# ZhicengShi/mclSTExp

Hardware: AMD Instinct MI355X
Metric: training spots/sec (= steps/sec x global batch) at batch 128/GPU, 224px patches, 1000 genes (higher is better)
Workload: dtype bf16; 1 GPU; BASELINE configs[1]: train step, batch 128/GPU, 224x224 patches, 1000 genes, densenet121 image encoder; global_batch=128, parallelism=dp1, backbone_dtype=bf16, infonce=fused, infonce_effective=exact (fused from 1024 pairs), hip_graphs=True, optimizer=Adam(lr=1e-4, wd=1e-3) incl. 2x(65536,G) tables

## Files before the change

mclstexp_amd/csrc/dense_bwd.hip:

```cpp
#include "common.h"
#include <stdlib.h>

namespace {

constexpr int TN = 128, TK = 128;

template <int MODE, int TMv>
__global__ __launch_bounds__(256, (TMv == 64 && MODE != 2 ? 3 : 2)) void bn1_bwd_kernel(const bf16_t* __restrict__ dz, const bf16_t* __restrict__ W1,
                                                         int K , int ldw ,
                                                         const bf16_t* __restrict__ x, long long ldx, long long S,
                                                         const float* __restrict__ gamma,
                                                         const float* __restrict__ beta,
                                                         const float* __restrict__ mean,
                                                         const float* __restrict__ rstd,
                                                         const float* __restrict__ coef ,
                                                         bf16_t* gbuf, long long ldg,
                                                         float2* __restrict__ partial , int nrt) {
  __shared__ __attribute__((aligned(16))) unsigned char lds[TK * 256 + TMv * 256 + 2048];
  const int tid = threadIdx.x, lane = tid & 63, wave = tid >> 6;
  const int h = lane >> 5, l31 = lane & 31;
  const int wm = wave >> 1, wn = wave & 1;
  const int n0 = blockIdx.y * TN;
  unsigned char* wt = lds;
  unsigned char* dzt = lds + TK * 256;
  bf16_t* xt = reinterpret_cast<bf16_t*>(dzt);
  float* red = reinterpret_cast<float*>(lds + TK * 256 + TMv * 256);

  const int cc = tid & 15, rr = tid >> 4;
  const bool cok = n0 + cc * 8 < K;
  constexpr int NL = TMv / 16, RI = TMv / 64;
  uint4 dzr[NL], xr[NL], gr[NL];
  auto issue_loads = [&](int rt) {
    const long long row0 = (long long)rt * TMv;
#pragma unroll
    for (int i = 0; i < NL; ++i) {
      const long long rg = row0 + rr + 16 * i;
      const bool ok = rg < S;
      dzr[i] = ok ? *reinterpret_cast<const uint4*>(dz + rg * TK + cc * 8) : make_uint4(0u, 0u, 0u, 0u);
      xr[i] = (ok && cok) ? *reinterpret_cast<const uint4*>(x + rg * ldx + n0 + cc * 8) : make_uint4(0u, 0u, 0u, 0u);
      if (MODE >= 1)
        gr[i] = (ok && cok) ? *reinterpret_cast<const uint4*>(gbuf + rg * ldg + n0 + cc * 8) : make_uint4(0u, 0u, 0u, 0u);
    }
  };
  if ((int)blockIdx.x < nrt) issue_loads(blockIdx.x);
  {
    uint4 wv[8];
#pragma unroll
    for (int i = 0; i < 8; ++i) {
      const int k = rr + 16 * i;
      wv[i] = cok ? *reinterpret_cast<const uint4*>(W1 + (long long)k * ldw + n0 + cc * 8) : make_uint4(0u, 0u, 0u, 0u);
    }
#pragma unroll
    for (int i = 0; i < 8; ++i) {
      const int k = rr + 16 * i;
      const int f = ((k & 3) << 2) | ((k >> 2) & 3);
      *reinterpret_cast<uint4*>(wt + k * 256 + ((cc ^ f) << 4)) = wv[i];
    }
  }
  float mu[2], rs[2], sc[2], sh[2], c1[2], c2[2];
#pragma unroll
  for (int j = 0; j < 2; ++j) {
    const int c = n0 + wn * 64 + j * 32 + l31;
    const bool cvalid = c < K;
    mu[j] = cvalid ? mean[c] : 0.0f;
    rs[j] = cvalid ? rstd[c] : 0.0f;
    sc[j] = cvalid ? gamma[c] * rs[j] : 0.0f;
    sh[j] = cvalid ? fmaf(-mu[j], sc[j], beta[c]) : 0.0f;
    c1[j] = (MODE >= 1 && coef != nullptr && cvalid) ? coef[2 * c] : 0.0f;
    c2[j] = (MODE >= 1 && coef != nullptr && cvalid) ? coef[2 * c + 1] : 0.0f;
  }
  const int q = (lane & 15) >> 2, jj = lane & 3;
  const int g2 = 2 * ((lane >> 4) & 1) + (jj >> 1);

  for (int rt = blockIdx.x; rt < nrt; rt += gridDim.x) {
    const long long row0 = (long long)rt * TMv;
    if (rt != (int)blockIdx.x) issue_loads(rt);
    __syncthreads();
#pragma unroll
    for (int i = 0; i < NL; ++i) {
      const int r = rr + 16 * i;
      *reinterpret_cast<uint4*>(dzt + r * 256 + ((cc ^ (r & 15)) << 4)) = dzr[i];
    }
    __syncthreads();

    f32x16 acc[RI][2];
#pragma unroll
    for (int i = 0; i < RI; ++i)
#pragma unroll
      for (int j = 0; j < 2; ++j)
#pragma unroll
        for (int r = 0; r < 16; ++r) acc[i][j][r] = 0.0f;
#pragma unroll
    for (int ks = 0; ks < 8; ++ks) {
      bf16x8 fa[RI], fb[2];
#pragma unroll
      for (int i = 0; i < RI; ++i) {
        const int r = wm * (TMv / 2) + i * 32 + l31;
        fa[i] = *reinterpret_cast<const bf16x8*>(dzt + r * 256 + (((2 * ks + h) ^ (r & 15)) << 4));
      }
#pragma unroll
      for (int j = 0; j < 2; ++j) {
        const int chunk = (wn * 64 + j * 32) / 8 + g2;
        const int k_lo = 16 * ks + 8 * h + q, k_hi = k_lo + 4;
        const int f_lo = ((k_lo & 3) << 2) | ((k_lo >> 2) & 3), f_hi = ((k_hi & 3) << 2) | ((k_hi >> 2) & 3);
        const v4s lo = __builtin_amdgcn_ds_read_tr16_b64_v4i16(
            (v4s __attribute__((address_space(3)))*)(wt + k_lo * 256 + ((chunk ^ f_lo) << 4) + (jj & 1) * 8));
        const v4s hi = __builtin_amdgcn_ds_read_tr16_b64_v4i16(
            (v4s __attribute__((address_space(3)))*)(wt + k_hi * 256 + ((chunk ^ f_hi) << 4) + (jj & 1) * 8));
        fb[j][0] = lo[0]; fb[j][1] = lo[1]; fb[j][2] = lo[2]; fb[j][3] = lo[3];
        fb[j][4] = hi[0]; fb[j][5] = hi[1]; fb[j][6] = hi[2]; fb[j][7] = hi[3];
      }
#pragma unroll
      for (int i = 0; i < RI; ++i)
#pragma unroll
        for (int j = 0; j < 2; ++j) acc[i][j] = __builtin_amdgcn_mfma_f32_32x32x16_bf16(fa[i], fb[j], acc[i][j], 0, 0, 0);
    }
    __syncthreads();
#pragma unroll
    for (int i = 0; i < NL; ++i) *reinterpret_cast<uint4*>(xt + (rr + 16 * i) * TN + cc * 8) = xr[i];
    __syncthreads();

    const long long nvalid = min((long long)TMv, S - row0);
    float s1[2], s2[2];
#pragma unroll
    for (int j = 0; j < 2; ++j) {
      const int cl = wn * 64 + j * 32 + l31;
      s1[j] = s2[j] = 0.0f;
      const float ka = MODE == 2 ? -c2[j] * rs[j] : -sc[j] * c2[j] * rs[j];
      const float kb = fmaf(-ka, mu[j], MODE == 2 ? -c1[j] : -sc[j] * c1[j]);
#pragma unroll
      for (int i = 0; i < RI; ++i)
#pragma unroll
        for (int r = 0; r < 16; ++r) {
          const int row = wm * (TMv / 2) + i * 32 + (r & 3) + 8 * (r >> 2) + 4 * h;
          const float xv = bf2f(xt[row * TN + cl]);
          const float gi = fmaf(xv, sc[j], sh[j]) > 0.0f ? acc[i][j][r] : 0.0f;
          if (MODE != 1) {
            if (row < nvalid) {
              s1[j] += gi;
              s2[j] = fmaf(gi, xv, s2[j]);
            }
          }
          if (MODE >= 1) xt[row * TN + cl] = f2bf(fmaf(sc[j], gi, fmaf(ka, xv, kb)));
        }
      if (MODE != 1) s2[j] = rs[j] * fmaf(-mu[j], s1[j], s2[j]);
    }
    if (MODE != 1) {
#pragma unroll
      for (int j = 0; j < 2; ++j) {
        s1[j] += __shfl_xor(s1[j], 32, 64);
        s2[j] += __shfl_xor(s2[j], 32, 64);
        if (h == 0) {
          const int cl = wn * 64 + j * 32 + l31;
          red[(wm * 128 + cl) * 2] = s1[j];
          red[(wm * 128 + cl) * 2 + 1] = s2[j];
        }
      }
      __syncthreads();
      if (tid < 128 && n0 + tid < K)
        partial[(long long)(n0 + tid) * nrt + rt] = make_float2(red[tid * 2] + red[(128 + tid) * 2],
                                                                red[tid * 2 + 1] + red[(128 + tid) * 2 + 1]);
    }
    if (MODE >= 1) {
      if (MODE == 1) __syncthreads();
      if (cok) {
#pragma unroll
        for (int i = 0; i < NL; ++i) {
          const int r = rr + 16 * i;
          const long long rg = row0 + r;
          if (rg < S) {
            const uint4 dv = *reinterpret_cast<const uint4*>(xt + r * TN + cc * 8);
            const unsigned gw[4] = {gr[i].x, gr[i].y, gr[i].z, gr[i].w}, dw[4] = {dv.x, dv.y, dv.z, dv.w};
            unsigned o[4];
#pragma unroll
            for (int u = 0; u < 4; ++u) {
              const float lo = __uint_as_float(gw[u] << 16) + __uint_as_float(dw[u] << 16);
              const float hi = __uint_as_float(gw[u] & 0xFFFF0000u) + __uint_as_float(dw[u] & 0xFFFF0000u);
              const f32x2 pv = {lo, hi};
              o[u] = __builtin_bit_cast(unsigned, __builtin_convertvector(pv, bf16x2_t));
            }
            *reinterpret_cast<uint4*>(gbuf + rg * ldg + n0 + cc * 8) = make_uint4(o[0], o[1], o[2], o[3]);
          }
        }
      }
    }
  }
}

constexpr size_t PAIR_LDS = 2 * TK * 256 + 64 * 256;
__global__ __launch_bounds__(256, 2) void bn1_dx_pair_kernel(const bf16_t* __restrict__ dzA, const bf16_t* __restrict__ W1A, int ldwA,
                                                             const float* __restrict__ gammaA, const float* __restrict__ betaA,
                                                             const float* __restrict__ coefA, const bf16_t* __restrict__ dzB,
                                                             const bf16_t* __restrict__ W1B, const float* __restrict__ gammaB,
                                                             const float* __restrict__ betaB, const float* __restrict__ coefB,
                                                             int K, const bf16_t* __restrict__ x, long long ldx, long long S,
                                                             const float* __restrict__ mean, const float* __restrict__ rstd,
                                                             bf16_t* gbuf, long long ldg, int nrt) {
  constexpr int TMv = 64;
  extern __shared__ __attribute__((aligned(16))) unsigned char lds[];
  const int tid = threadIdx.x, lane = tid & 63, wave = tid >> 6;
  const int h = lane >> 5, l31 = lane & 31;
  const int wm = wave >> 1, wn = wave & 1;
  const int n0 = blockIdx.y * TN;
  unsigned char* wtA = lds;
  unsigned char* wtB = lds + TK * 256;
  unsigned char* dzt = lds + 2 * TK * 256;
  bf16_t* xt = reinterpret_cast<bf16_t*>(dzt);
  const int cc = tid & 15, rr = tid >> 4;
  const bool cok = n0 + cc * 8 < K;
  constexpr int NL = TMv / 16;
  uint4 dar[NL], dbr[NL], xr[NL], gr[NL];
  auto issue_loads = [&](int rt) {
    const long long row0 = (long long)rt * TMv;
#pragma unroll
    for (int i = 0; i < NL; ++i) {
      const long long rg = row0 + rr + 16 * i;
      const bool ok = rg < S;
      dar[i] = ok ? *reinterpret_cast<const uint4*>(dzA + rg * TK + cc * 8) : make_uint4(0u, 0u, 0u, 0u);
      dbr[i] = ok ? *reinterpret_cast<const uint4*>(dzB + rg * TK + cc * 8) : make_uint4(0u, 0u, 0u, 0u);
      xr[i] = (ok && cok) ? *reinterpret_cast<const uint4*>(x + rg * ldx + n0 + cc * 8) : make_uint4(0u, 0u, 0u, 0u);
      gr[i] = (ok && cok) ? *reinterpret_cast<const uint4*>(gbuf + rg * ldg + n0 + cc * 8) : make_uint4(0u, 0u, 0u, 0u);
    }
  };
  if ((int)blockIdx.x < nrt) issue_loads(blockIdx.x);
  {
    uint4 wa[8], wb[8];
#pragma unroll
    for (int i = 0; i < 8; ++i) {
      const int k = rr + 16 * i;
      wa[i] = cok ? *reinterpret_cast<const uint4*>(W1A + (long long)k * ldwA + n0 + cc * 8) : make_uint4(0u, 0u, 0u, 0u);
      wb[i] = cok ? *reinterpret_cast<const uint4*>(W1B + (long long)k * K + n0 + cc * 8) : make_uint4(0u, 0u, 0u, 0u);
    }
#pragma unroll
    for (int i = 0; i < 8; ++i) {
      const int k = rr + 16 * i;
      const int f = ((k & 3) << 2) | ((k >> 2) & 3);
      *reinterpret_cast<uint4*>(wtA + k * 256 + ((cc ^ f) << 4)) = wa[i];
      *reinterpret_cast<uint4*>(wtB + k * 256 + ((cc ^ f) << 4)) = wb[i];
    }
  }
  float scA[2], shA[2], scB[2], shB[2], ka[2], kb[2];
#pragma unroll
  for (int j = 0; j < 2; ++j) {
    const int c = n0 + wn * 64 + j * 32 + l31;
    const bool cv = c < K;
    const float mu = cv ? mean[c] : 0.0f, rs = cv ? rstd[c] : 0.0f;
    scA[j] = cv ? gammaA[c] * rs : 0.0f;
    shA[j] = cv ? fmaf(-mu, scA[j], betaA[c]) : 0.0f;
    scB[j] = cv ? gammaB[c] * rs : 0.0f;
    shB[j] = cv ? fmaf(-mu, scB[j], betaB[c]) : 0.0f;
    const float c1A = cv ? coefA[2 * c] : 0.0f, c2A = cv ? coefA[2 * c + 1] : 0.0f;
    const float c1B = cv ? coefB[2 * c] : 0.0f, c2B = cv ? coefB[2 * c + 1] : 0.0f;
    const float kaA = -scA[j] * c2A * rs, kaB = -scB[j] * c2B * rs;
    const float kbA = fmaf(-kaA, mu, -scA[j] * c1A), kbB = fmaf(-kaB, mu, -scB[j] * c1B);
    ka[j] = kaA + kaB;
    kb[j] = kbA + kbB;
  }
  const int q = (lane & 15) >> 2, jj = lane & 3;
  const int g2 = 2 * ((lane >> 4) & 1) + (jj >> 1);
  auto product = [&](const unsigned char* wt, f32x16 (&acc)[2]) {
#pragma unroll
    for (int j = 0; j < 2; ++j)
#pragma unroll
      for (int r = 0; r < 16; ++r) acc[j][r] = 0.0f;
#pragma unroll
    for (int ks = 0; ks < 8; ++ks) {
      const int r = wm * (TMv / 2) + l31;
      const bf16x8 fa = *reinterpret_cast<const bf16x8*>(dzt + r * 256 + (((2 * ks + h) ^ (r & 15)) << 4));
      bf16x8 fb[2];
#pragma unroll
      for (int j = 0; j < 2; ++j) {
        const int chunk = (wn * 64 + j * 32) / 8 + g2;
        const int k_lo = 16 * ks + 8 * h + q, k_hi = k_lo + 4;
        const int f_lo = ((k_lo & 3) << 2) | ((k_lo >> 2) & 3), f_hi = ((k_hi & 3) << 2) | ((k_hi >> 2) & 3);
        const v4s lo = __builtin_amdgcn_ds_read_tr16_b64_v4i16(
            (v4s __attribute__((address_space(3)))*)(wt + k_lo * 256 + ((chunk ^ f_lo) << 4) + (jj & 1) * 8));
        const v4s hi = __builtin_amdgcn_ds_read_tr16_b64_v4i16(
            (v4s __attribute__((address_space(3)))*)(wt + k_hi * 256 + ((chunk ^ f_hi) << 4) + (jj & 1) * 8));
        fb[j][0] = lo[0]; fb[j][1] = lo[1]; fb[j][2] = lo[2]; fb[j][3] = lo[3];
        fb[j][4] = hi[0]; fb[j][5] = hi[1]; fb[j][6] = hi[2]; fb[j][7] = hi[3];
      }
#pragma unroll
      for (int j = 0; j < 2; ++j) acc[j] = __builtin_amdgcn_mfma_f32_32x32x16_bf16(fa, fb[j], acc[j], 0, 0, 0);
    }
  };
  for (int rt = blockIdx.x; rt < nrt; rt += gridDim.x) {
    const long long row0 = (long long)rt * TMv;
    if (rt != (int)blockIdx.x) issue_loads(rt);
    __syncthreads();
#pragma unroll
    for (int i = 0; i < NL; ++i) {
      const int r = rr + 16 * i;
      *reinterpret_cast<uint4*>(dzt + r * 256 + ((cc ^ (r & 15)) << 4)) = dar[i];
    }
    __syncthreads();
    f32x16 accA[2], accB[2];
    product(wtA, accA);
    __syncthreads();
#pragma unroll
    for (int i = 0; i < NL; ++i) {
      const int r = rr + 16 * i;
      *reinterpret_cast<uint4*>(dzt + r * 256 + ((cc ^ (r & 15)) << 4)) = dbr[i];
    }
    __syncthreads();
    product(wtB, accB);
    __syncthreads();
#pragma unroll
    for (int i = 0; i < NL; ++i) *reinterpret_cast<uint4*>(xt + (rr + 16 * i) * TN + cc * 8) = xr[i];
    __syncthreads();
#pragma unroll
    for (int j = 0; j < 2; ++j) {
      const int cl = wn * 64 + j * 32 + l31;
#pragma unroll
      for (int r = 0; r < 16; ++r) {
        const int row = wm * (TMv / 2) + (r & 3) + 8 * (r >> 2) + 4 * h;
        const float xv = bf2f(xt[row * TN + cl]);
        const float gA = fmaf(xv, scA[j], shA[j]) > 0.0f ? accA[j][r] : 0.0f;
        const float gB = fmaf(xv, scB[j], shB[j]) > 0.0f ? accB[j][r] : 0.0f;
        xt[row * TN + cl] = f2bf(fmaf(scA[j], gA, fmaf(scB[j], gB, fmaf(ka[j], xv, kb[j]))));
      }
    }
    __syncthreads();
    if (cok) {
#pragma unroll
      for (int i = 0; i < NL; ++i) {
        const int r = rr + 16 * i;
        const long long rg = row0 + r;
        if (rg < S) {
          const uint4 dv = *reinterpret_cast<const uint4*>(xt + r * TN + cc * 8);
          const unsigned gw[4] = {gr[i].x, gr[i].y, gr[i].z, gr[i].w}, dw[4] = {dv.x, dv.y, dv.z, dv.w};
          unsigned o[4];
#pragma unroll
          for (int u = 0; u < 4; ++u) {
            const float lo = __uint_as_float(gw[u] << 16) + __uint_as_float(dw[u] << 16);
            const float hi = __uint_as_float(gw[u] & 0xFFFF0000u) + __uint_as_float(dw[u] & 0xFFFF0000u);
            const f32x2 pv = {lo, hi};
            o[u] = __builtin_bit_cast(unsigned, __builtin_convertvector(pv, bf16x2_t));
          }
          *reinterpret_cast<uint4*>(gbuf + rg * ldg + n0 + cc * 8) = make_uint4(o[0], o[1], o[2], o[3]);
        }
      }
    }
  }
}

__global__ __launch_bounds__(256) void bn1_bwd_finalize_kernel(const float2* __restrict__ partial, int nrt, int C,
                                                               long long S, float* __restrict__ dgamma,
                                                               float* __restrict__ dbeta, float* __restrict__ coef,
                                                               int accumulate_params,
                                                               float* __restrict__ kacc = nullptr ,
                                                               const float* __restrict__ gamma = nullptr,
                                                               const float* __restrict__ rstd = nullptr) {
  __shared__ double red[2][4];
  const int c = blockIdx.x, lane = threadIdx.x & 63, wave = threadIdx.x >> 6;
  const float2* p = partial + (long long)c * nrt;
  double a = 0.0, b = 0.0;
  constexpr int U = 8;
  for (int t0 = threadIdx.x; t0 < nrt; t0 += 256 * U) {
    float2 v[U];
#pragma unroll
    for (int u = 0; u < U; ++u) v[u] = p[min(t0 + 256 * u, nrt - 1)];
#pragma unroll
    for (int u = 0; u < U; ++u) {
      if (t0 + 256 * u >= nrt) v[u] = make_float2(0.0f, 0.0f);
      a += (double)v[u].x;
      b += (double)v[u].y;
    }
  }
#pragma unroll
  for (int o = 32; o > 0; o >>= 1) {
    a += __shfl_xor(a, o, 64);
    b += __shfl_xor(b, o, 64);
  }
  if (lane == 0) {
    red[0][wave] = a;
    red[1][wave] = b;
  }
  __syncthreads();
  if (threadIdx.x != 0) return;
  a = (red[0][0] + red[0][1]) + (red[0][2] + red[0][3]);
  b = (red[1][0] + red[1][1]) + (red[1][2] + red[1][3]);
  if (accumulate_params) {
    dbeta[c] += (float)a;
    dgamma[c] += (float)b;
  } else {
    dbeta[c] = (float)a;
    dgamma[c] = (float)b;
  }
  if (kacc != nullptr) {
    const double scv = (double)gamma[c] * (double)rstd[c];
    kacc[2 * c] = (float)(scv * a / (double)S);
    kacc[2 * c + 1] = (float)(scv * b / (double)S);
    return;
  }
  coef[2 * c] = (float)(a / (double)S);
  coef[2 * c + 1] = (float)(b / (double)S);
}

__global__ __launch_bounds__(256) void bn1_fix_kernel(const bf16_t* __restrict__ x, long long ldx, bf16_t* __restrict__ gbuf,
                                                      long long ldg, long long S, int c0, int nc,
                                                      const float* __restrict__ mean, const float* __restrict__ rstd,
                                                      const float* __restrict__ kacc) {
  const int cpr = nc >> 3;
  const long long n = S * cpr;
  const long long i0 = (long long)blockIdx.x * 256 + threadIdx.x, istride = (long long)gridDim.x * 256;
  const bool fixed = (istride % cpr) == 0;
  uint4 xv = make_uint4(0u, 0u, 0u, 0u), gv = xv;
  if (i0 < n) {
    const long long row = i0 / cpr;
    const int c = c0 + (int)(i0 - row * cpr) * 8;
    xv = *reinterpret_cast<const uint4*>(x + row * ldx + c);
    gv = *reinterpret_cast<const uint4*>(gbuf + row * ldg + c);
  }
  float kav[8], kbv[8];
  auto consts = [&](int c) {
#pragma unroll
    for (int e = 0; e < 8; ++e) {
      const float k1 = kacc[2 * (c + e)], k2 = kacc[2 * (c + e) + 1];
      kav[e] = k2 * rstd[c + e];
      kbv[e] = fmaf(-kav[e], mean[c + e], k1);
    }
  };
  if (i0 < n) consts(c0 + (int)(i0 % cpr) * 8);
  for (long long i = i0; i < n; i += istride) {
    const long long row = i / cpr;
    const int c = c0 + (int)(i - row * cpr) * 8;
    if (i != i0) {
      xv = *reinterpret_cast<const uint4*>(x + row * ldx + c);
      gv = *reinterpret_cast<const uint4*>(gbuf + row * ldg + c);
      if (!fixed) consts(c);
    }
    const unsigned xw[4] = {xv.x, xv.y, xv.z, xv.w};
    unsigned gw[4] = {gv.x, gv.y, gv.z, gv.w};
#pragma unroll
    for (int u = 0; u < 4; ++u) {
      float o[2];
#pragma unroll
      for (int e = 0; e < 2; ++e) {
        const float ka = kav[2 * u + e], kb = kbv[2 * u + e];
        const float xf = e ? __uint_as_float(xw[u] & 0xFFFF0000u) : __uint_as_float(xw[u] << 16);
        const float gf = e ? __uint_as_float(gw[u] & 0xFFFF0000u) : __uint_as_float(gw[u] << 16);
        o[e] = gf - fmaf(ka, xf, kb);
      }
      const f32x2 pv = {o[0], o[1]};
      gw[u] = __builtin_bit_cast(unsigned, __builtin_convertvector(pv, bf16x2_t));
    }
    *reinterpret_cast<uint4*>(gbuf + row * ldg + c) = make_uint4(gw[0], gw[1], gw[2], gw[3]);
  }
}

constexpr int C3I = 128, C3O = 32, T3B = 128;

__global__ __launch_bounds__(256, 1) void conv3x3_bwd_kernel(const bf16_t* __restrict__ dy, long long lddy, long long S,
                                                             int H, int W, const bf16_t* __restrict__ W2,
                                                             const bf16_t* __restrict__ z,
                                                             const float* __restrict__ gamma,
                                                             const float* __restrict__ beta,
                                                             const float* __restrict__ mean,
                                                             const float* __restrict__ rstd, bf16_t* __restrict__ g2,
                                                             float2* __restrict__ partial, int ntile,
                                                             const bf16_t* __restrict__ xfix, long long ldxf,
                                                             const float* __restrict__ fmean,
                                                             const float* __restrict__ frstd,
                                                             const float* __restrict__ fk, bf16_t* __restrict__ dyc) {
  extern __shared__ __attribute__((aligned(16))) unsigned char lds[];
  const int tid = threadIdx.x, lane = tid & 63, wave = tid >> 6;
  const int h = lane >> 5, l31 = lane & 31;
  const int nrow = T3B + 2 * W + 2;
  bf16_t* zt = reinterpret_cast<bf16_t*>(lds);
  unsigned char* slab = lds + T3B * 256;
  const int zero_off = T3B * 256 + nrow * 64;
  const int Si = (int)S;

  uint4 zr[8];
  auto load_z_tile = [&](int tile) {
    const int p0 = tile * T3B;
#pragma unroll
    for (int i = 0; i < 8; ++i) {
      const int p = p0 + (tid >> 4) + 16 * i;
      zr[i] = p < Si ? *reinterpret_cast<const uint4*>(z + (long long)p * C3I + (tid & 15) * 8) : make_uint4(0u, 0u, 0u, 0u);
    }
  };
  if ((int)blockIdx.x < ntile) load_z_tile(blockIdx.x);
  bf16x8 breg[18];
#pragma unroll
  for (int i = 0; i < 18; ++i) {
    const int tap = i >> 1, co0 = 16 * (i & 1) + 8 * h;
#pragma unroll
    for (int j = 0; j < 8; ++j)
      breg[i][j] = (short)W2[((long long)(co0 + j) * 9 + tap) * C3I + 32 * wave + l31];
  }
  const int c = 32 * wave + l31;
  const float mu = mean[c], rs = rstd[c];
  const float sc = gamma[c] * rs, sh = fmaf(-mu, sc, beta[c]);
  int abase[18];
#pragma unroll
  for (int i = 0; i < 18; ++i) {
    const int tap = i >> 1, ky = tap / 3, kx = tap % 3;
    const int row = l31 + (2 - ky) * W + (2 - kx);
    abase[i] = T3B * 256 + row * 64 + (((2 * (i & 1) + h) ^ ((row >> 2) & 3)) << 4);
  }
  if (tid < 4) *reinterpret_cast<uint4*>(lds + zero_off + tid * 16) = make_uint4(0u, 0u, 0u, 0u);
  float fka[8], fkb[8];
  if (xfix != nullptr) {
#pragma unroll
    for (int e = 0; e < 8; ++e) {
      const int cf = (tid & 3) * 8 + e;
      const float k1 = fk[2 * cf], k2 = fk[2 * cf + 1];
      fka[e] = k2 * frstd[cf];
      fkb[e] = fmaf(-fka[e], fmean[cf], k1);
    }
  }

  for (int tile = blockIdx.x; tile < ntile; tile += gridDim.x) {
    const int p0 = tile * T3B;
    if (tile != (int)blockIdx.x) load_z_tile(tile);
    __syncthreads();
    for (int q = tid; q < nrow * 4; q += 256) {
      const int j = q >> 2, ch = q & 3;
      const int p = p0 - (W + 1) + j;
      uint4 v = make_uint4(0u, 0u, 0u, 0u);
      if (p >= 0 && p < Si) {
        v = *reinterpret_cast<const uint4*>(dy + (long long)p * lddy + ch * 8);
        if (xfix != nullptr) {
          const uint4 xv = *reinterpret_cast<const uint4*>(xfix + (long long)p * ldxf + ch * 8);
          const unsigned xw[4] = {xv.x, xv.y, xv.z, xv.w};
          unsigned gw[4] = {v.x, v.y, v.z, v.w};
#pragma unroll
          for (int u = 0; u < 4; ++u) {
            const float o_lo = __uint_as_float(gw[u] << 16) - fmaf(fka[2 * u], __uint_as_float(xw[u] << 16), fkb[2 * u]);
            const float o_hi = __uint_as_float(gw[u] & 0xFFFF0000u) -
                               fmaf(fka[2 * u + 1], __uint_as_float(xw[u] & 0xFFFF0000u), fkb[2 * u + 1]);
            const f32x2 pv = {o_lo, o_hi};
            gw[u] = __builtin_bit_cast(unsigned, __builtin_convertvector(pv, bf16x2_t));
          }
          v = make_uint4(gw[0], gw[1], gw[2], gw[3]);
          if (dyc != nullptr && j >= W + 1 && j < W + 1 + T3B) *reinterpret_cast<uint4*>(dyc + (long long)p * C3O + ch * 8) = v;
        }
      }
      *reinterpret_cast<uint4*>(slab + j * 64 + ((ch ^ ((j >> 2) & 3)) << 4)) = v;
    }
#pragma unroll
    for (int i = 0; i < 8; ++i)
      *reinterpret_cast<uint4*>(zt + ((tid >> 4) + 16 * i) * C3I + (tid & 15) * 8) = zr[i];
    unsigned vmask[4];
#pragma unroll
    for (int mb = 0; mb < 4; ++mb) {
      const int p = p0 + mb * 32 + l31;
      const int x = p % W, y = (p / W) % H;
      unsigned m = 0;
      if (p < Si) {
#pragma unroll
        for (int ky = 0; ky < 3; ++ky)
#pragma unroll
          for (int kx = 0; kx < 3; ++kx) {
            const int yy = y + 1 - ky, xx = x + 1 - kx;
            if (yy >= 0 && yy < H && xx >= 0 && xx < W) m |= 1u << (ky * 3 + kx);
          }
      }
      vmask[mb] = m;
    }
    f32x16 acc[4];
#pragma unroll
    for (int mb = 0; mb < 4; ++mb)
#pragma unroll
      for (int r = 0; r < 16; ++r) acc[mb][r] = 0.0f;
    __syncthreads();

#pragma unroll
    for (int i = 0; i < 18; ++i) {
#pragma unroll
      for (int mb = 0; mb < 4; ++mb) {
        const int off = ((vmask[mb] >> (i >> 1)) & 1u) ? abase[i] + mb * 2048 : zero_off;
        const bf16x8 a = *reinterpret_cast<const bf16x8*>(lds + off);
        acc[mb] = __builtin_amdgcn_mfma_f32_32x32x16_bf16(a, breg[i], acc[mb], 0, 0, 0);
      }
    }
    const int nvalid = min(T3B, Si - p0);
    float s1 = 0.0f, s2 = 0.0f;
#pragma unroll
    for (int mb = 0; mb < 4; ++mb)
#pragma unroll
      for (int r = 0; r < 16; ++r) {
        const int px = mb * 32 + (r & 3) + 8 * (r >> 2) + 4 * h;
        const float zv = bf2f(zt[px * C3I + c]);
        const float gi = fmaf(zv, sc, sh) > 0.0f ? acc[mb][r] : 0.0f;
        const bf16_t gb = f2bf(gi);
        if (px < nvalid) {
          const float gr_ = bf2f(gb);
          s1 += gr_;
          s2 = fmaf(gr_, (zv - mu) * rs, s2);
        }
        zt[px * C3I + c] = gb;
      }
    s1 += __shfl_xor(s1, 32, 64);
    s2 += __shfl_xor(s2, 32, 64);
    if (h == 0) partial[(long long)c * ntile + tile] = make_float2(s1, s2);
    __syncthreads();
#pragma unroll
    for (int i = 0; i < 8; ++i) {
      const int r = (tid >> 4) + 16 * i;
      const int p = p0 + r;
      if (p < Si)
        *reinterpret_cast<uint4*>(g2 + (long long)p * C3I + (tid & 15) * 8) =
            *reinterpret_cast<const uint4*>(zt + r * C3I + (tid & 15) * 8);
    }
  }
}

constexpr int BR_NWAVE = 8;
constexpr int BR_SLOT = 34 * 64;
constexpr int BR_RING = 4 * BR_SLOT;

__device__ __forceinline__ void br_swap8(unsigned (&w)[8]) {
#pragma unroll
  for (int g = 0; g < 2; ++g)
#pragma unroll
    for (int d = 0; d < 2; ++d) {
      const u32x2 r = __builtin_amdgcn_permlane32_swap(w[4 * g + d], w[4 * g + 2 + d], false, false);
      w[4 * g + d] = r[0];
      w[4 * g + 2 + d] = r[1];
    }
}

template <bool K0, bool K2>
__device__ __forceinline__ void br_row_mfma(const unsigned char* __restrict__ ring, int jo, const int (&foff)[3][2],
                                            const bf16x8 (&breg)[18], f32x16& acc) {
  constexpr int KY0 = K0 ? 0 : 1, KY1 = K2 ? 3 : 2, NT = (KY1 - KY0) * 3;
  f32x16 acc2;
#pragma unroll
  for (int r = 0; r < 16; ++r) acc2[r] = 0.0f;
  bf16x8 b[2][2];
  auto fetch = [&](int t, int buf) {
    const int ky = KY0 + t / 3, kx = t % 3;
    const unsigned char* slot = ring + ((jo + 1 - ky) & 3) * BR_SLOT;
    b[buf][0] = *reinterpret_cast<const bf16x8*>(slot + foff[kx][0]);
    b[buf][1] = *reinterpret_cast<const bf16x8*>(slot + foff[kx][1]);
  };
  fetch(0, 0);
#pragma unroll
  for (int t = 0; t < NT; ++t) {
    const int cur = t & 1, tap = (KY0 + t / 3) * 3 + t % 3;
    if (t + 1 < NT) fetch(t + 1, cur ^ 1);
    __builtin_amdgcn_sched_barrier(0);
    acc = __builtin_amdgcn_mfma_f32_32x32x16_bf16(breg[tap * 2], b[cur][0], acc, 0, 0, 0);
// ... 462 lines not shown
```

Baseline: 12120 spots/s.

## Prefetch next row tile in BN backward kernels and use unconditional clamped loads

Restructures the bn1 backward and paired dx kernels so that, once each operand's current tile has been staged to LDS, the operand for the next row tile is loaded into registers, overlapping global loads with MFMA and epilogue work. Loads are made unconditional by clamping row and column addresses, with masking applied at the LDS store (keep4). Per-channel parameter loads are hoisted ahead of the weight loads and blocks with no work exit early. This adds register pressure and some redundant clamped loads at tile edges, which could reduce occupancy.

After: 12430 spots/s (median of 6 runs). 1.03x the previous value.

```diff
diff --git a/mclstexp_amd/csrc/dense_bwd.hip b/mclstexp_amd/csrc/dense_bwd.hip
--- a/mclstexp_amd/csrc/dense_bwd.hip
+++ b/mclstexp_amd/csrc/dense_bwd.hip
@@ -4,6 +4,10 @@
 namespace {
 
 constexpr int TN = 128, TK = 128;
+
+__device__ __forceinline__ uint4 keep4(bool keep, const uint4 v) {
+  return make_uint4(keep ? v.x : 0u, keep ? v.y : 0u, keep ? v.z : 0u, keep ? v.w : 0u);
+}
 
 template <int MODE, int TMv>
 __global__ __launch_bounds__(256, (TMv == 64 && MODE != 2 ? 3 : 2)) void bn1_bwd_kernel(const bf16_t* __restrict__ dz, const bf16_t* __restrict__ W1,
@@ -28,59 +32,79 @@
 
   const int cc = tid & 15, rr = tid >> 4;
   const bool cok = n0 + cc * 8 < K;
+  if ((int)blockIdx.x >= nrt) return;
   constexpr int NL = TMv / 16, RI = TMv / 64;
+  constexpr bool PF = MODE != 0;
+  const int colc = cok ? n0 + cc * 8 : n0;
   uint4 dzr[NL], xr[NL], gr[NL];
-  auto issue_loads = [&](int rt) {
-    const long long row0 = (long long)rt * TMv;
-#pragma unroll
-    for (int i = 0; i < NL; ++i) {
-      const long long rg = row0 + rr + 16 * i;
-      const bool ok = rg < S;
-      dzr[i] = ok ? *reinterpret_cast<const uint4*>(dz + rg * TK + cc * 8) : make_uint4(0u, 0u, 0u, 0u);
-      xr[i] = (ok && cok) ? *reinterpret_cast<const uint4*>(x + rg * ldx + n0 + cc * 8) : make_uint4(0u, 0u, 0u, 0u);
-      if (MODE >= 1)
-        gr[i] = (ok && cok) ? *reinterpret_cast<const uint4*>(gbuf + rg * ldg + n0 + cc * 8) : make_uint4(0u, 0u, 0u, 0u);
-    }
+  auto rowc = [&](long long base, bool spread, int i) { return spread ? min(base + rr + 16 * i, S - 1) : base; };
+  auto load_dz = [&](long long base, bool spread) {
+#pragma unroll
+    for (int i = 0; i < NL; ++i) dzr[i] = *reinterpret_cast<const uint4*>(dz + rowc(base, spread, i) * TK + cc * 8);
   };
-  if ((int)blockIdx.x < nrt) issue_loads(blockIdx.x);
+  auto load_x = [&](long long base, bool spread) {
+#pragma unroll
+    for (int i = 0; i < NL; ++i) xr[i] = *reinterpret_cast<const uint4*>(x + rowc(base, spread, i) * ldx + colc);
+  };
+  auto load_g = [&](long long base, bool spread) {
+#pragma unroll
+    for (int i = 0; i < NL; ++i) gr[i] = *reinterpret_cast<const uint4*>(gbuf + rowc(base, spread, i) * ldg + colc);
+  };
+  const bool hc = MODE >= 1 && coef != nullptr;
+  float mu[2], rs[2], gm[2], bt[2], c1[2], c2[2];
+#pragma unroll
+  for (int j = 0; j < 2; ++j) {
+    const int c = min(n0 + wn * 64 + j * 32 + l31, K - 1);
+    mu[j] = mean[c];
+    rs[j] = rstd[c];
+    gm[j] = gamma[c];
+    bt[j] = beta[c];
+    if (MODE >= 1) {
+      const float* cp = hc ? coef + 2 * c : mean + c;
+      c1[j] = cp[0];
+      c2[j] = cp[hc ? 1 : 0];
+    }
+  }
+  load_dz((long long)blockIdx.x * TMv, true);
   {
     uint4 wv[8];
 #pragma unroll
-    for (int i = 0; i < 8; ++i) {
-      const int k = rr + 16 * i;
-      wv[i] = cok ? *reinterpret_cast<const uint4*>(W1 + (long long)k * ldw + n0 + cc * 8) : make_uint4(0u, 0u, 0u, 0u);
-    }
+    for (int i = 0; i < 8; ++i) wv[i] = *reinterpret_cast<const uint4*>(W1 + (long long)(rr + 16 * i) * ldw + colc);
+    load_x((long long)blockIdx.x * TMv, true);
+    if (MODE >= 1) load_g((long long)blockIdx.x * TMv, true);
 #pragma unroll
     for (int i = 0; i < 8; ++i) {
       const int k = rr + 16 * i;
       const int f = ((k & 3) << 2) | ((k >> 2) & 3);
-      *reinterpret_cast<uint4*>(wt + k * 256 + ((cc ^ f) << 4)) = wv[i];
-    }
-  }
-  float mu[2], rs[2], sc[2], sh[2], c1[2], c2[2];
+      *reinterpret_cast<uint4*>(wt + k * 256 + ((cc ^ f) << 4)) = keep4(cok, wv[i]);
+    }
+  }
+  float sc[2], sh[2];
 #pragma unroll
   for (int j = 0; j < 2; ++j) {
-    const int c = n0 + wn * 64 + j * 32 + l31;
-    const bool cvalid = c < K;
-    mu[j] = cvalid ? mean[c] : 0.0f;
-    rs[j] = cvalid ? rstd[c] : 0.0f;
-    sc[j] = cvalid ? gamma[c] * rs[j] : 0.0f;
-    sh[j] = cvalid ? fmaf(-mu[j], sc[j], beta[c]) : 0.0f;
-    c1[j] = (MODE >= 1 && coef != nullptr && cvalid) ? coef[2 * c] : 0.0f;
-    c2[j] = (MODE >= 1 && coef != nullptr && cvalid) ? coef[2 * c + 1] : 0.0f;
+    const bool cvalid = n0 + wn * 64 + j * 32 + l31 < K;
+    mu[j] = cvalid ? mu[j] : 0.0f;
+    rs[j] = cvalid ? rs[j] : 0.0f;
+    sc[j] = cvalid ? gm[j] * rs[j] : 0.0f;
+    sh[j] = cvalid ? fmaf(-mu[j], sc[j], bt[j]) : 0.0f;
+    c1[j] = (hc && cvalid) ? c1[j] : 0.0f;
+    c2[j] = (hc && cvalid) ? c2[j] : 0.0f;
   }
   const int q = (lane & 15) >> 2, jj = lane & 3;
   const int g2 = 2 * ((lane >> 4) & 1) + (jj >> 1);
 
   for (int rt = blockIdx.x; rt < nrt; rt += gridDim.x) {
     const long long row0 = (long long)rt * TMv;
-    if (rt != (int)blockIdx.x) issue_loads(rt);
+    const bool more = rt + (int)gridDim.x < nrt;
+    const long long nbase = more ? row0 + (long long)gridDim.x * TMv : row0;
+    if (!PF && rt != (int)blockIdx.x) { load_dz(row0, true); load_x(row0, true); if (MODE >= 1) load_g(row0, true); }
     __syncthreads();
 #pragma unroll
     for (int i = 0; i < NL; ++i) {
       const int r = rr + 16 * i;
-      *reinterpret_cast<uint4*>(dzt + r * 256 + ((cc ^ (r & 15)) << 4)) = dzr[i];
-    }
+      *reinterpret_cast<uint4*>(dzt + r * 256 + ((cc ^ (r & 15)) << 4)) = keep4(row0 + r < S, dzr[i]);
+    }
+    if (PF) load_dz(nbase, more);
     __syncthreads();
 
     f32x16 acc[RI][2];
@@ -117,7 +141,9 @@
     }
     __syncthreads();
 #pragma unroll
-    for (int i = 0; i < NL; ++i) *reinterpret_cast<uint4*>(xt + (rr + 16 * i) * TN + cc * 8) = xr[i];
+    for (int i = 0; i < NL; ++i)
+      *reinterpret_cast<uint4*>(xt + (rr + 16 * i) * TN + cc * 8) = keep4(cok && row0 + rr + 16 * i < S, xr[i]);
+    if (PF) load_x(nbase, more);
     __syncthreads();
 
     const long long nvalid = min((long long)TMv, S - row0);
@@ -183,6 +209,7 @@
           }
         }
       }
+      if (PF) load_g(nbase, more);
     }
   }
 }
@@ -209,48 +236,74 @@
   const int cc = tid & 15, rr = tid >> 4;
   const bool cok = n0 + cc * 8 < K;
   constexpr int NL = TMv / 16;
+  if ((int)blockIdx.x >= nrt) return;
+  const int colc = cok ? n0 + cc * 8 : n0;
   uint4 dar[NL], dbr[NL], xr[NL], gr[NL];
-  auto issue_loads = [&](int rt) {
-    const long long row0 = (long long)rt * TMv;
-#pragma unroll
-    for (int i = 0; i < NL; ++i) {
-      const long long rg = row0 + rr + 16 * i;
-      const bool ok = rg < S;
-      dar[i] = ok ? *reinterpret_cast<const uint4*>(dzA + rg * TK + cc * 8) : make_uint4(0u, 0u, 0u, 0u);
-      dbr[i] = ok ? *reinterpret_cast<const uint4*>(dzB + rg * TK + cc * 8) : make_uint4(0u, 0u, 0u, 0u);
-      xr[i] = (ok && cok) ? *reinterpret_cast<const uint4*>(x + rg * ldx + n0 + cc * 8) : make_uint4(0u, 0u, 0u, 0u);
-      gr[i] = (ok && cok) ? *reinterpret_cast<const uint4*>(gbuf + rg * ldg + n0 + cc * 8) : make_uint4(0u, 0u, 0u, 0u);
-    }
+  auto rowc = [&](long long base, bool spread, int i) { return spread ? min(base + rr + 16 * i, S - 1) : base; };
+  auto load_dzA = [&](long long base, bool spread) {
+#pragma unroll
+    for (int i = 0; i < NL; ++i) dar[i] = *reinterpret_cast<const uint4*>(dzA + rowc(base, spread, i) * TK + cc * 8);
   };
-  if ((int)blockIdx.x < nrt) issue_loads(blockIdx.x);
+  auto load_dzB = [&](long long base, bool spread) {
+#pragma unroll
+    for (int i = 0; i < NL; ++i) dbr[i] = *reinterpret_cast<const uint4*>(dzB + rowc(base, spread, i) * TK + cc * 8);
+  };
+  auto load_x = [&](long long base, bool spread) {
+#pragma unroll
+    for (int i = 0; i < NL; ++i) xr[i] = *reinterpret_cast<const uint4*>(x + rowc(base, spread, i) * ldx + colc);
+  };
+  auto load_g = [&](long long base, bool spread) {
+#pragma unroll
+    for (int i = 0; i < NL; ++i) gr[i] = *reinterpret_cast<const uint4*>(gbuf + rowc(base, spread, i) * ldg + colc);
+  };
+  float mur[2], rsr[2], gA[2], bA[2], gB[2], bB[2], cA[2][2], cB[2][2];
+#pragma unroll
+  for (int j = 0; j < 2; ++j) {
+    const int c = min(n0 + wn * 64 + j * 32 + l31, K - 1);
+    mur[j] = mean[c];
+    rsr[j] = rstd[c];
+    gA[j] = gammaA[c];
+    bA[j] = betaA[c];
+    gB[j] = gammaB[c];
+    bB[j] = betaB[c];
+    cA[j][0] = coefA[2 * c];
+    cA[j][1] = coefA[2 * c + 1];
+    cB[j][0] = coefB[2 * c];
+    cB[j][1] = coefB[2 * c + 1];
+  }
+  __builtin_amdgcn_sched_barrier(0);
   {
     uint4 wa[8], wb[8];
 #pragma unroll
     for (int i = 0; i < 8; ++i) {
       const int k = rr + 16 * i;
-      wa[i] = cok ? *reinterpret_cast<const uint4*>(W1A + (long long)k * ldwA + n0 + cc * 8) : make_uint4(0u, 0u, 0u, 0u);
-      wb[i] = cok ? *reinterpret_cast<const uint4*>(W1B + (long long)k * K + n0 + cc * 8) : make_uint4(0u, 0u, 0u, 0u);
-    }
+      wa[i] = *reinterpret_cast<const uint4*>(W1A + (long long)k * ldwA + colc);
+      wb[i] = *reinterpret_cast<const uint4*>(W1B + (long long)k * K + colc);
+    }
+    load_dzA((long long)blockIdx.x * TMv, true);
+    load_dzB((long long)blockIdx.x * TMv, true);
+    load_x((long long)blockIdx.x * TMv, true);
+    load_g((long long)blockIdx.x * TMv, true);
+    __builtin_amdgcn_sched_barrier(0);
 #pragma unroll
     for (int i = 0; i < 8; ++i) {
       const int k = rr + 16 * i;
       const int f = ((k & 3) << 2) | ((k >> 2) & 3);
-      *reinterpret_cast<uint4*>(wtA + k * 256 + ((cc ^ f) << 4)) = wa[i];
-      *reinterpret_cast<uint4*>(wtB + k * 256 + ((cc ^ f) << 4)) = wb[i];
+      *reinterpret_cast<uint4*>(wtA + k * 256 + ((cc ^ f) << 4)) = keep4(cok, wa[i]);
+      *reinterpret_cast<uint4*>(wtB + k * 256 + ((cc ^ f) << 4)) = keep4(cok, wb[i]);
     }
   }
   float scA[2], shA[2], scB[2], shB[2], ka[2], kb[2];
 #pragma unroll
   for (int j = 0; j < 2; ++j) {
-    const int c = n0 + wn * 64 + j * 32 + l31;
-    const bool cv = c < K;
-    const float mu = cv ? mean[c] : 0.0f, rs = cv ? rstd[c] : 0.0f;
-    scA[j] = cv ? gammaA[c] * rs : 0.0f;
-    shA[j] = cv ? fmaf(-mu, scA[j], betaA[c]) : 0.0f;
-    scB[j] = cv ? gammaB[c] * rs : 0.0f;
-    shB[j] = cv ? fmaf(-mu, scB[j], betaB[c]) : 0.0f;
-    const float c1A = cv ? coefA[2 * c] : 0.0f, c2A = cv ? coefA[2 * c + 1] : 0.0f;
-    const float c1B = cv ? coefB[2 * c] : 0.0f, c2B = cv ? coefB[2 * c + 1] : 0.0f;
+    const bool cv = n0 + wn * 64 + j * 32 + l31 < K;
+    const float mu = cv ? mur[j] : 0.0f, rs = cv ? rsr[j] : 0.0f;
+    scA[j] = cv ? gA[j] * rs : 0.0f;
+    shA[j] = cv ? fmaf(-mu, scA[j], bA[j]) : 0.0f;
+    scB[j] = cv ? gB[j] * rs : 0.0f;
+    shB[j] = cv ? fmaf(-mu, scB[j], bB[j]) : 0.0f;
+    const float c1A = cv ? cA[j][0] : 0.0f, c2A = cv ? cA[j][1] : 0.0f;
+    const float c1B = cv ? cB[j][0] : 0.0f, c2B = cv ? cB[j][1] : 0.0f;
     const float kaA = -scA[j] * c2A * rs, kaB = -scB[j] * c2B * rs;
     const float kbA = fmaf(-kaA, mu, -scA[j] * c1A), kbB = fmaf(-kaB, mu, -scB[j] * c1B);
     ka[j] = kaA + kaB;
@@ -286,13 +339,15 @@
   };
   for (int rt = blockIdx.x; rt < nrt; rt += gridDim.x) {
     const long long row0 = (long long)rt * TMv;
-    if (rt != (int)blockIdx.x) issue_loads(rt);
+    const bool more = rt + (int)gridDim.x < nrt;
+    const long long nbase = more ? row0 + (long long)gridDim.x * TMv : row0;
     __syncthreads();
 #pragma unroll
     for (int i = 0; i < NL; ++i) {
       const int r = rr + 16 * i;
-      *reinterpret_cast<uint4*>(dzt + r * 256 + ((cc ^ (r & 15)) << 4)) = dar[i];
-    }
+      *reinterpret_cast<uint4*>(dzt + r * 256 + ((cc ^ (r & 15)) << 4)) = keep4(row0 + r < S, dar[i]);
+    }
+    load_dzA(nbase, more);
     __syncthreads();
     f32x16 accA[2], accB[2];
     product(wtA, accA);
@@ -300,13 +355,16 @@
 #pragma unroll
     for (int i = 0; i < NL; ++i) {
       const int r = rr + 16 * i;
-      *reinterpret_cast<uint4*>(dzt + r * 256 + ((cc ^ (r & 15)) << 4)) = dbr[i];
-    }
+      *reinterpret_cast<uint4*>(dzt + r * 256 + ((cc ^ (r & 15)) << 4)) = keep4(row0 + r < S, dbr[i]);
+    }
+    load_dzB(nbase, more);
     __syncthreads();
     product(wtB, accB);
     __syncthreads();
 #pragma unroll
-    for (int i = 0; i < NL; ++i) *reinterpret_cast<uint4*>(xt + (rr + 16 * i) * TN + cc * 8) = xr[i];
+    for (int i = 0; i < NL; ++i)
+      *reinterpret_cast<uint4*>(xt + (rr + 16 * i) * TN + cc * 8) = keep4(cok && row0 + rr + 16 * i < S, xr[i]);
+    load_x(nbase, more);
     __syncthreads();
 #pragma unroll
     for (int j = 0; j < 2; ++j) {
@@ -341,6 +399,7 @@
         }
       }
     }
+    load_g(nbase, more);
   }
 }
 
```
